# js43o/HifiDiff

Hardware: AMD Instinct MI355X
Metric: faces/sec (whole node), 16→128 1000-step reverse diffusion, batch 64 (higher is better)
Workload: dtype bf16

## Files before the change

hifidiff_amd/csrc/hd_xcd.hpp:

```cpp
#pragma once
#include <type_traits>
#ifndef HD_XCD_ROWS
#define HD_XCD_ROWS 0
#endif
#if HD_XCD_ROWS
#define HD_XCD_KERNEL xcd_rows_stage_kernel
#define HD_XCD_LAUNCH launch_xcd_rows_stage
#else
#define HD_XCD_KERNEL xcd_stage_kernel
#define HD_XCD_LAUNCH launch_xcd_stage
#endif

#include "hd_gemm.hpp"
#include "hd_stage_api.hpp"

#ifndef HD_XS_W0
#define HD_XS_W0 0
#endif
#ifndef HD_XS_READY
#define HD_XS_READY 1
#endif
#ifndef HD_XS_PUBFIRST
#define HD_XS_PUBFIRST 1
#endif
#ifndef HD_XS_WNT
#define HD_XS_WNT 0
#endif

#pragma clang fp contract(off)

namespace hd {

template <int C_, int HW_>
struct XcdCfg {
    static constexpr int C = C_, HW = HW_;
    static constexpr int R = XS_FACES * HW;
    static constexpr int NT = C / 32;
    static constexpr int RSPLIT = XS_GROUP_WG / NT;
    static constexpr int RCU = R / RSPLIT;
    static constexpr int WMW = RCU / 32;
    static constexpr int WK = 8 / WMW;
    static constexpr int CPW = C / 64 / WK;
    static constexpr int KS = C / 16;
    static constexpr int FCU = RCU / HW;
    static constexpr int S = (HW == 4) ? 2 : (HW == 16) ? 4 : (HW == 64) ? 8 : (HW == 256) ? 16 : 1;
    static constexpr int TPR = XS_THREADS / RCU;
    static constexpr int NIT = RCU * 32 / XS_THREADS;
    static constexpr int A_WAVE = 32 * LDS_ROW;
    static constexpr bool kStoresFirst = C_ >= 1024;
    static_assert(RSPLIT * NT == XS_GROUP_WG && WMW * WK == 8 && CPW == 2 && S * S == HW, "geometry");
    static_assert(RCU / S * 32 == XS_THREADS, "one (channel, image row) item per thread in the depthwise epilogue");
    static_assert(TPR * 4 >= NT, "partials per thread");
};

template <int C, int HW, int GBF = 1>
struct XLds {
    typedef XcdCfg<C, HW> K;
    char stage[K::WK * K::RCU * 32 * 2 * 4];
    float xt[K::RCU * 32], yt[K::RCU * 32];
    unsigned short gt[K::RCU * 32];
    float rs[(K::RCU / K::S) * 32];
    float pl[XS_FACES * 32];
    float2 stats[K::RCU];
    float gb[GBF * 2 * C];
    float dwc[22 * 32];
    XBlockW blk[XS_MAXBLK];
    unsigned base, local, abort, pad_;
};

typedef __attribute__((address_space(1))) unsigned xs_gu32;
typedef unsigned xs_u32x4 __attribute__((ext_vector_type(4)));
typedef unsigned xs_u32x2 __attribute__((ext_vector_type(2)));

__device__ __forceinline__ unsigned xs_xcc_id() {
    unsigned v;
    asm volatile("s_getreg_b32 %0, hwreg(HW_REG_XCC_ID)" : "=s"(v));
    return v & 0xfu;
}
__device__ __forceinline__ uint4 xs_ldg_u4(const uint4* p) {
#if HD_XS_WNT
    const xs_u32x4 v = __builtin_nontemporal_load(reinterpret_cast<__attribute__((address_space(1))) const xs_u32x4*>((unsigned long long)p));
#else
    const xs_u32x4 v = *reinterpret_cast<__attribute__((address_space(1))) const xs_u32x4*>((unsigned long long)p);
#endif
    return make_uint4(v.x, v.y, v.z, v.w);
}
__device__ __forceinline__ float xs_ldg_f(const float* p) { return *reinterpret_cast<__attribute__((address_space(1))) const float*>((unsigned long long)p); }
__device__ __forceinline__ float4 xs_ldg_f4(const float* p) {
    typedef float f4v __attribute__((ext_vector_type(4)));
    const f4v v = *reinterpret_cast<__attribute__((address_space(1))) const f4v*>((unsigned long long)p);
    return make_float4(v.x, v.y, v.z, v.w);
}
__device__ __forceinline__ void xs_ready(float& x) {
#if HD_XS_READY
    asm volatile("" : "+v"(x));
#endif
}
__device__ __forceinline__ void xs_lds_barrier() { asm volatile("s_waitcnt lgkmcnt(0)\n\ts_barrier" ::: "memory"); }

#ifdef HD_STAMPS
#define HD_XSTAMP(i) do { if (p.stamps && tid == 0) p.stamps[((size_t)ph * 256 + blockIdx.x) * 8 + (i)] = __builtin_amdgcn_s_memrealtime(); } while (0)
#else
#define HD_XSTAMP(i) do { } while (0)
#endif

template <int C, int HW>
__global__ __launch_bounds__(XS_THREADS) void HD_XCD_KERNEL(const XStageP p) {
    typedef XcdCfg<C, HW> K;
    __shared__ __attribute__((aligned(16))) XLds<C, HW, HD_XCD_ROWS ? XcdCfg<C, HW>::FCU : 1> L;
    const int tid = threadIdx.x, lane = tid & 63, wave = __builtin_amdgcn_readfirstlane(tid >> 6);
    const int group = blockIdx.x & 7, rank = blockIdx.x >> 3;
    const int face_g0 = group * XS_FACES;
    if (face_g0 >= p.B) return;
    const int ct = rank % K::NT, rsp = rank / K::NT;
    const int M = p.B * HW;
    const int row0 = face_g0 * HW + rsp * K::RCU;
    const int face0 = row0 / HW;
    const int wm = wave / K::WK, wk = wave - wm * K::WK;
    const int c0 = wk * K::CPW;
    const int kq = lane & 7;
    const int col = ct * 32 + (tid & 31);

    {
        const unsigned* src = reinterpret_cast<const unsigned*>(p.blocks);
        unsigned* dst = reinterpret_cast<unsigned*>(L.blk);
        for (int i = tid; i < p.nblocks * (int)(sizeof(XBlockW) / 4); i += XS_THREADS) dst[i] = src[i];
        if (tid == 0) L.abort = __hip_atomic_load((xs_gu32*)p.abort_dev, __ATOMIC_RELAXED, __HIP_MEMORY_SCOPE_AGENT);
    }
    xs_lds_barrier();

#ifdef HD_STAMPS
    const size_t act_bytes = p.dbg_no_a ? 0 : (size_t)M * C * 2;
#else
    const size_t act_bytes = (size_t)M * C * 2;
#endif
    const __amdgpu_buffer_rsrc_t rs_Xb = __builtin_amdgcn_make_buffer_rsrc(p.Xb, 0, (int)act_bytes, 0x00020000);
    const __amdgpu_buffer_rsrc_t rs_Yb = __builtin_amdgcn_make_buffer_rsrc(p.Yb, 0, (int)act_bytes, 0x00020000);
    const __amdgpu_buffer_rsrc_t rs_G = __builtin_amdgcn_make_buffer_rsrc(p.G, 0, (int)act_bytes, 0x00020000);
    const __amdgpu_buffer_rsrc_t rs_P16 = __builtin_amdgcn_make_buffer_rsrc(p.pooled16, 0, p.B * C * 2, 0x00020000);
    const __amdgpu_buffer_rsrc_t rs_sx = __builtin_amdgcn_make_buffer_rsrc(p.sx, 0, M * K::NT * 8, 0x00020000);
    const __amdgpu_buffer_rsrc_t rs_sy = __builtin_amdgcn_make_buffer_rsrc(p.sy, 0, M * K::NT * 8, 0x00020000);

    uint4 bq[K::CPW][4][2];
    xs_u32x4 aq[K::CPW][4];
    f32x16_t acc[2];

    auto load_w_chunk = [&](const uint4* W, auto pair_c, auto d_c) __attribute__((always_inline)) {
        constexpr bool PAIR = decltype(pair_c)::value;
        constexpr int d = decltype(d_c)::value;
#ifdef HD_STAMPS
        if (p.dbg_no_w) return;
#endif
        const uint4* Wl = W + lane;
#pragma unroll
        for (int ss = 0; ss < 4; ++ss) {
            bq[d][ss][0] = xs_ldg_u4(Wl + ((size_t)ct * K::KS + (c0 + d) * 4 + ss) * 64);
            if (PAIR) bq[d][ss][1] = xs_ldg_u4(Wl + ((size_t)(ct + K::NT) * K::KS + (c0 + d) * 4 + ss) * 64);
        }
    };
    auto load_w = [&](const uint4* W, auto pair_c) __attribute__((always_inline)) {
        load_w_chunk(W, pair_c, std::integral_constant<int, 0>());
        load_w_chunk(W, pair_c, std::integral_constant<int, 1>());
    };
    auto load_a = [&](const __amdgpu_buffer_rsrc_t& rs) __attribute__((always_inline)) {
#pragma unroll
        for (int d = 0; d < K::CPW; ++d)
#pragma unroll
            for (int u = 0; u < 4; ++u) {
                const int gr = row0 + wm * 32 + (lane >> 3) + 8 * u;
                const int r = gr < M ? gr : 0;
                aq[d][u] = __builtin_amdgcn_raw_buffer_load_b128(rs, (r * C + (c0 + d) * 64 + 8 * kq) * 2, 0, 16);
            }
    };
    char* sA = L.stage + wave * K::A_WAVE;
    const int a_lane_off = (lane & 31) * LDS_ROW + (lane >> 5) * 16;
    auto zero_acc = [&]() __attribute__((always_inline)) {
#pragma unroll
        for (int tn = 0; tn < 2; ++tn)
#pragma unroll
            for (int i = 0; i < 16; ++i) acc[tn][i] = 0.f;
    };
    auto chunk_mma = [&](int d, auto pair_c) __attribute__((always_inline)) {
        constexpr bool PAIR = decltype(pair_c)::value;
        __builtin_amdgcn_wave_barrier();
#pragma unroll
        for (int ss = 0; ss < 4; ++ss) {
            const bf16x8_t a = *reinterpret_cast<const bf16x8_t*>(sA + a_lane_off + ss * 32);
            acc[0] = __builtin_amdgcn_mfma_f32_32x32x16_bf16(a, __builtin_bit_cast(bf16x8_t, bq[d][ss][0]), acc[0], 0, 0, 0);
            if (PAIR) acc[1] = __builtin_amdgcn_mfma_f32_32x32x16_bf16(a, __builtin_bit_cast(bf16x8_t, bq[d][ss][1]), acc[1], 0, 0, 0);
        }
        __builtin_amdgcn_wave_barrier();
    };
    auto gemm_plain = [&](auto pair_c) __attribute__((always_inline)) {
        zero_acc();
#pragma unroll
        for (int d = 0; d < K::CPW; ++d) {
#pragma unroll
            for (int u = 0; u < 4; ++u) {
                const int gr = row0 + wm * 32 + (lane >> 3) + 8 * u;
                const xs_u32x4 v = gr < M ? aq[d][u] : (xs_u32x4){0u, 0u, 0u, 0u};
                *reinterpret_cast<xs_u32x4*>(sA + ((lane >> 3) + 8 * u) * LDS_ROW + 16 * kq) = v;
            }
            chunk_mma(d, pair_c);
        }
    };
    auto gemm_ln = [&]() __attribute__((always_inline)) {
        zero_acc();
        f32x2_t rsv[4], muv[4];
#pragma unroll
        for (int u = 0; u < 4; ++u) {
            float2 s = L.stats[wm * 32 + (lane >> 3) + 8 * u];
            asm volatile("s_waitcnt lgkmcnt(0)\n\ts_nop 3" : "+v"(s.x), "+v"(s.y));
            const float mu = -s.x * s.y;
            rsv[u] = (f32x2_t){s.y, s.y}; muv[u] = (f32x2_t){mu, mu};
        }
#pragma unroll
        for (int d = 0; d < K::CPW; ++d) {
            const int k = (c0 + d) * 64 + 8 * kq;
            f32x2_t g[4], b[4];
#if !HD_XCD_ROWS
#pragma unroll
            for (int i = 0; i < 4; ++i) {
                g[i] = *reinterpret_cast<const f32x2_t*>(&L.gb[k + 2 * i]);
                b[i] = *reinterpret_cast<const f32x2_t*>(&L.gb[C + k + 2 * i]);
            }
#endif
#pragma unroll
            for (int u = 0; u < 4; ++u) {
#if HD_XCD_ROWS
                {
                    const float* gbf = &L.gb[((wm * 32 + (lane >> 3) + 8 * u) / HW) * 2 * C];
#pragma unroll
                    for (int i = 0; i < 4; ++i) {
                        g[i] = *reinterpret_cast<const f32x2_t*>(&gbf[k + 2 * i]);
                        b[i] = *reinterpret_cast<const f32x2_t*>(&gbf[C + k + 2 * i]);
                    }
                }
#endif
                const unsigned w[4] = {aq[d][u].x, aq[d][u].y, aq[d][u].z, aq[d][u].w};
                unsigned o[4];
#pragma unroll
                for (int i = 0; i < 4; ++i) {
                    const f32x2_t x = {__uint_as_float(w[i] << 16), __uint_as_float(w[i] & 0xffff0000u)};
                    o[i] = pack2(__builtin_elementwise_fma(__builtin_elementwise_fma(x, rsv[u], muv[u]), g[i], b[i]));
                }
                *reinterpret_cast<xs_u32x4*>(sA + ((lane >> 3) + 8 * u) * LDS_ROW + 16 * kq) = (xs_u32x4){o[0], o[1], o[2], o[3]};
            }
            chunk_mma(d, std::true_type());
        }
    };
    float* red = reinterpret_cast<float*>(L.stage);
    auto to_red = [&](auto pair_c) __attribute__((always_inline)) {
        constexpr int TNT = decltype(pair_c)::value ? 2 : 1;
        constexpr int TILE_F = K::RCU * 32 * TNT;
        xs_lds_barrier();
#pragma unroll
        for (int tn = 0; tn < TNT; ++tn)
#pragma unroll
            for (int i = 0; i < 16; ++i) {
                const int r = wm * 32 + (i & 3) + 8 * (i >> 2) + 4 * (lane >> 5);
                red[wk * TILE_F + (tn * K::RCU + r) * 32 + (lane & 31)] = acc[tn][i];
            }
        xs_lds_barrier();
    };
    float2 ln_ps[4];
    float4 ln_g = make_float4(0.f, 0.f, 0.f, 0.f), ln_b = ln_g;
#if HD_XCD_ROWS
    int ln_film_off = 0;
#endif
    auto ln_issue = [&](const __amdgpu_buffer_rsrc_t& rs, int film_bias_off) __attribute__((always_inline)) {
        constexpr int TPR = K::TPR;
        const int rl = tid / TPR, part = tid % TPR, row = row0 + rl;
        const bool rv = row < M;
#pragma unroll
        for (int i = 0; i < 4; ++i) {
            const int j = part + i * TPR;
            ln_ps[i] = make_float2(0.f, -1.f);
            if (rv && j < K::NT) {
                const xs_u32x2 raw = __builtin_amdgcn_raw_buffer_load_b64(rs, (row * K::NT + j) * 8, 0, 16);
                ln_ps[i] = make_float2(__uint_as_float(raw.x), __uint_as_float(raw.y));
            }
        }
        static_assert(C <= XS_THREADS * 4, "one float4 of gain and bias per thread");
        const int k = tid * 4;
#if HD_XCD_ROWS
        ln_film_off = film_bias_off;
        (void)k;
#else
        if (k < C) {
            ln_b = *reinterpret_cast<const float4*>(p.film + film_bias_off + k);
            ln_g = *reinterpret_cast<const float4*>(p.film + film_bias_off + C + k);
        }
#endif
    };
    auto ln_finish = [&]() __attribute__((always_inline)) {
        constexpr int TPR = K::TPR;
        const int rl = tid / TPR, part = tid % TPR;
        const bool rv = row0 + rl < M;
        const int k = tid * 4;
#if HD_XCD_ROWS
        (void)ln_g; (void)ln_b; (void)k;
        for (int q = tid; q < K::FCU * (C / 4); q += XS_THREADS) {
            const int f = q / (C / 4), kk = (q - f * (C / 4)) * 4;
            const int face = (face0 + f) < p.B ? face0 + f : 0;
            const float* src = p.film + (size_t)face * p.film_face_stride + ln_film_off;
            *reinterpret_cast<float4*>(&L.gb[f * 2 * C + kk]) = *reinterpret_cast<const float4*>(src + C + kk);
            *reinterpret_cast<float4*>(&L.gb[f * 2 * C + C + kk]) = *reinterpret_cast<const float4*>(src + kk);
        }
#else
        if (k < C) {
            *reinterpret_cast<float4*>(&L.gb[k]) = ln_g;
            *reinterpret_cast<float4*>(&L.gb[C + k]) = ln_b;
        }
#endif
        auto row_sum = [](float v) __attribute__((always_inline)) {
            if (TPR > 1) v += dpp_mov<0xB1>(v);
            if (TPR > 2) v += dpp_mov<0x4E>(v);
            if (TPR > 4) v += dpp_mov<0x141>(v);
            if (TPR > 8) v += dpp_mov<0x140>(v);
            return v;
        };
        float sm = 0.f;
#pragma unroll
        for (int i = 0; i < 4; ++i) sm += ln_ps[i].y >= 0.f ? ln_ps[i].x : 0.f;
        const float inv_np = 1.0f / (float)K::NT;
        const float mean = row_sum(sm) * inv_np;
        const float cnt = 32.f;
        float q = 0.f;
#pragma unroll
        for (int i = 0; i < 4; ++i) {
            const float d = ln_ps[i].x - mean;
            q += ln_ps[i].y >= 0.f ? fmaf(cnt * d, d, ln_ps[i].y) : 0.f;
        }
        const float var = row_sum(q) * (inv_np / cnt);
        if (part == 0) L.stats[rl] = make_float2(mean, rv ? __frsqrt_rn(var + p.ln_eps) : 0.f);
        xs_lds_barrier();
    };
    bool local = false;
    auto st128 = [&](const __amdgpu_buffer_rsrc_t& rs, int off, uint4 v) __attribute__((always_inline)) {
        const xs_u32x4 x = {v.x, v.y, v.z, v.w};
        if (local) __builtin_amdgcn_raw_buffer_store_b128(x, rs, off, 0, 0);
        else __builtin_amdgcn_raw_buffer_store_b128(x, rs, off, 0, 16);
    };
    auto st64 = [&](const __amdgpu_buffer_rsrc_t& rs, int off, float2 v) __attribute__((always_inline)) {
        const xs_u32x2 x = {__float_as_uint(v.x), __float_as_uint(v.y)};
        if (local) __builtin_amdgcn_raw_buffer_store_b64(x, rs, off, 0, 0);
        else __builtin_amdgcn_raw_buffer_store_b64(x, rs, off, 0, 16);
    };
    xs_gu32* flags = (xs_gu32*)(p.flags + group * 32);
    unsigned base = 0;
    bool dead = false;
    auto publish = [&](int ph) __attribute__((always_inline)) {
        asm volatile("s_waitcnt vmcnt(0)" ::: "memory");
        if (lane == 0) {
            if (local) __hip_atomic_store(flags + rank, base + (unsigned)ph + 1u, __ATOMIC_RELAXED, __HIP_MEMORY_SCOPE_WORKGROUP);
            else __hip_atomic_store(flags + rank, base + (unsigned)ph + 1u, __ATOMIC_RELAXED, __HIP_MEMORY_SCOPE_AGENT);
        }
    };
    auto wait_phase = [&](int ph) __attribute__((always_inline)) {
        if (wave == 0) {
            const unsigned want = base + (unsigned)ph + 1u;
            for (unsigned spins = 0;; ++spins) {
                const unsigned v = lane < XS_GROUP_WG ? __hip_atomic_load(flags + lane, __ATOMIC_RELAXED, __HIP_MEMORY_SCOPE_AGENT) : want;
                const bool inject = p.test_abort > 0 && ph + 1 == p.test_abort && group == 0;
                if (!inject && __all((int)(v - want) >= 0)) break;
                if (spins > XS_SPINS || inject) {
                    if (lane == 0) {
                        L.abort = 1u;
                        __hip_atomic_store((xs_gu32*)p.abort_dev, 0x100u + (unsigned)ph, __ATOMIC_RELAXED, __HIP_MEMORY_SCOPE_AGENT);
                        __hip_atomic_store((xs_gu32*)p.tmo, 0x100u + (unsigned)ph, __ATOMIC_RELAXED, __HIP_MEMORY_SCOPE_SYSTEM);
                    }
                    break;
                }
                __builtin_amdgcn_s_sleep(1);
            }
        }
        xs_lds_barrier();
        dead = L.abort != 0u;
    };
    float2* st_out = L.stats;

    load_w(L.blk[0].w1, std::true_type());
    if (wave == 0) {
        xs_gu32* gs = (xs_gu32*)(p.gstate + group * 32);
        xs_gu32* hello = (xs_gu32*)(p.hello + group * 32);
        const unsigned n = __hip_atomic_load(gs, __ATOMIC_RELAXED, __HIP_MEMORY_SCOPE_AGENT);
        const unsigned xcc = xs_xcc_id();
        const unsigned mine = ((n + 1u) << 4) | xcc;
        if (lane == 0) __hip_atomic_store(hello + rank, mine, __ATOMIC_RELAXED, __HIP_MEMORY_SCOPE_AGENT);
        bool same = false;
        for (unsigned spins = 0;; ++spins) {
            const unsigned v = lane < XS_GROUP_WG ? __hip_atomic_load(hello + lane, __ATOMIC_RELAXED, __HIP_MEMORY_SCOPE_AGENT) : mine;
            if (__all((v >> 4) == (n + 1u))) { same = __all((v & 15u) == xcc); break; }
            if (spins > XS_SPINS) {
                if (lane == 0) {
                    L.abort = 1u;
                    __hip_atomic_store((xs_gu32*)p.abort_dev, 0x80u, __ATOMIC_RELAXED, __HIP_MEMORY_SCOPE_AGENT);
                    __hip_atomic_store((xs_gu32*)p.tmo, 0x80u, __ATOMIC_RELAXED, __HIP_MEMORY_SCOPE_SYSTEM);
                }
                break;
            }
            __builtin_amdgcn_s_sleep(1);
        }
        if (lane == 0) { L.base = n * 64u; L.local = (same && !p.force_global) ? 1u : 0u; }
    }
    for (int u = tid; u < K::RCU * 8; u += XS_THREADS) {
        const int r = u >> 3, q4 = u & 7;
        float4 v = make_float4(0.f, 0.f, 0.f, 0.f);
        if (row0 + r < M) v = *reinterpret_cast<const float4*>(p.X + (size_t)(row0 + r) * C + ct * 32 + q4 * 4);
        *reinterpret_cast<float4*>(&L.xt[r * 32 + q4 * 4]) = v;
    }
    xs_lds_barrier();
    if (L.abort) return;
    base = L.base; local = L.local != 0u;

    const int P = 5 * p.nblocks;
    const int P_run = (p.phase_limit > 0 && p.phase_limit < P) ? p.phase_limit : P;

    for (int blk = 0; blk < p.nblocks; ++blk) {
        const XBlockW& B = L.blk[blk];
        {
            const int ph = 5 * blk;
            if (ph >= P_run) break;
            HD_XSTAMP(0);
            if (ph > 0) { wait_phase(ph - 1); if (dead) return; }
            HD_XSTAMP(1);
            ln_issue(rs_sx, B.film_off);
            if (HD_XS_W0 == 0 && ph > 0 && wave == 0) load_w(B.w1, std::true_type());
            load_a(rs_Xb);
            float dwc[2];
#pragma unroll
            for (int i = 0; i < 2; ++i) {
                const int e = tid + i * XS_THREADS, k = e >> 5, cc = ct * 32 + (e & 31);
                dwc[i] = 0.f;
                if (k < 18) dwc[i] = xs_ldg_f(B.dw_w + (size_t)(k % 9) * 2 * C + cc + (k >= 9 ? C : 0));
                else if (k < 20) dwc[i] = xs_ldg_f(B.dw_b + cc + (k == 19 ? C : 0));
                else if (k < 22) dwc[i] = xs_ldg_f(B.b1 + cc + (k == 21 ? C : 0));
            }
            ln_finish();
            gemm_ln();
            if ((wave != 0 || HD_XS_W0 >= 2) && ph + 1 < P_run) load_w_chunk(B.wsca, std::false_type(), std::integral_constant<int, 0>());
            if (HD_XS_W0 == 2 && wave == 0 && ph + 1 < P_run) load_w_chunk(B.wsca, std::false_type(), std::integral_constant<int, 1>());
            HD_XSTAMP(2);
#pragma unroll
            for (int i = 0; i < 2; ++i) { const int e = tid + i * XS_THREADS; if (e < 22 * 32) L.dwc[e] = dwc[i]; }
            to_red(std::true_type());
            HD_XSTAMP(6);
            constexpr int TILE_F = K::RCU * 32 * 2;
            float dw_wa[9], dw_wb[9];
            const int jc = tid & 31;
#pragma unroll
            for (int t = 0; t < 9; ++t) { dw_wa[t] = L.dwc[t * 32 + jc]; dw_wb[t] = L.dwc[(9 + t) * 32 + jc]; }
            const float dw_ba = L.dwc[18 * 32 + jc], dw_bb = L.dwc[19 * 32 + jc], b1a = L.dwc[20 * 32 + jc], b1b = L.dwc[21 * 32 + jc];
            for (int e = tid; e < K::RCU * 32; e += XS_THREADS) {
                float va = b1a, vb = b1b;
#pragma unroll
                for (int w = 0; w < K::WK; ++w) { va += red[w * TILE_F + e]; vb += red[w * TILE_F + K::RCU * 32 + e]; }
                red[e] = va; red[K::RCU * 32 + e] = vb;
            }
            xs_lds_barrier();
            {
                const int j = tid & 31, rr = tid >> 5;
                constexpr int ls = (K::S == 2) ? 1 : (K::S == 4) ? 2 : (K::S == 8) ? 3 : (K::S == 16) ? 4 : 0;
                const int p0 = rr << ls;
                const int y = (p0 & (HW - 1)) >> ls;
                const float rsum = dw_gate_row<K::S>(red + j, red + K::RCU * 32 + j, p0, y > 0, y < K::S - 1, dw_wa, dw_wb, dw_ba, dw_bb,
                                                     L.gt + p0 * 32 + j, 32, true, K::S);
                L.rs[rr * 32 + j] = rsum;
            }
            xs_lds_barrier();
            if (tid < K::FCU * 32) {
                const int f = tid >> 5, j = tid & 31;
                float sacc = 0.f;
#pragma unroll
                for (int r = 0; r < K::S; ++r) sacc += L.rs[(f * K::S + r) * 32 + j];
                L.pl[f * 32 + j] = sacc / (float)HW;
            }
            xs_lds_barrier();
            if constexpr (!K::kStoresFirst) { if (wave != 0 && ph + 1 < P_run) load_w_chunk(B.wsca, std::false_type(), std::integral_constant<int, 1>()); }
            HD_XSTAMP(3);
            if (wave == 0) {
                if (lane < K::FCU * 4) {
                    const int f = lane >> 2, q4 = lane & 3;
                    if (face0 + f < p.B) {
                        st128(rs_P16, ((face0 + f) * C + ct * 32 + q4 * 8) * 2, pack8(&L.pl[f * 32 + q4 * 8]));
                        if (p.pooled) {
                            *reinterpret_cast<float4*>(p.pooled + (size_t)(face0 + f) * C + ct * 32 + q4 * 8) = *reinterpret_cast<const float4*>(&L.pl[f * 32 + q4 * 8]);
                            *reinterpret_cast<float4*>(p.pooled + (size_t)(face0 + f) * C + ct * 32 + q4 * 8 + 4) = *reinterpret_cast<const float4*>(&L.pl[f * 32 + q4 * 8 + 4]);
                        }
                    }
                }
                HD_XSTAMP(4);
            }
#if HD_XS_PUBFIRST
            if (wave == 0) publish(ph);
#endif
            if constexpr (K::kStoresFirst) xs_lds_barrier();
            if constexpr (K::kStoresFirst) { if (wave != 0 && ph + 1 < P_run) load_w_chunk(B.wsca, std::false_type(), std::integral_constant<int, 1>()); }
#if !HD_XS_PUBFIRST
            if (wave == 0) publish(ph);
#endif
            if (HD_XS_W0 == 1 && wave == 0 && ph + 1 < P_run) load_w(B.wsca, std::false_type());
            if (HD_XS_W0 == 3 && wave == 0 && ph + 1 < P_run) load_w_chunk(B.wsca, std::false_type(), std::integral_constant<int, 1>());
            HD_XSTAMP(5);
        }
        {
            const int ph = 5 * blk + 1;
            if (ph >= P_run) break;
            HD_XSTAMP(0);
            wait_phase(ph - 1); if (dead) return;
            if (HD_XS_W0 == 0 && wave == 0) load_w(B.wsca, std::false_type());
            HD_XSTAMP(1);
            float bsca = xs_ldg_f(B.bsca + col);
            zero_acc();
            if (wm == 0) {
                xs_u32x4 pa[K::CPW];
                const int f = lane >> 3;
                const bool fv = f < K::FCU && face0 + f < p.B;
#pragma unroll
                for (int d = 0; d < K::CPW; ++d)
                    pa[d] = __builtin_amdgcn_raw_buffer_load_b128(rs_P16, ((fv ? face0 + f : 0) * C + (c0 + d) * 64 + 8 * kq) * 2, 0, 16);
                for (int i = lane; i < 24 * LDS_ROW / 16; i += 64) reinterpret_cast<uint4*>(sA + 8 * LDS_ROW)[i] = make_uint4(0, 0, 0, 0);
#pragma unroll
                for (int d = 0; d < K::CPW; ++d) {
                    *reinterpret_cast<xs_u32x4*>(sA + f * LDS_ROW + 16 * kq) = fv ? pa[d] : (xs_u32x4){0u, 0u, 0u, 0u};
                    chunk_mma(d, std::false_type());
                }
            }
            xs_ready(bsca);
            if ((wave != 0 || HD_XS_W0 >= 2) && ph + 1 < P_run) load_w_chunk(B.w3, std::false_type(), std::integral_constant<int, 0>());
            if (HD_XS_W0 == 2 && wave == 0 && ph + 1 < P_run) load_w_chunk(B.w3, std::false_type(), std::integral_constant<int, 1>());
            HD_XSTAMP(2);
            xs_lds_barrier();
            if (wm == 0) {
#pragma unroll
                for (int i = 0; i < 16; ++i) {
                    const int r = (i & 3) + 8 * (i >> 2) + 4 * (lane >> 5);
                    if (r < XS_FACES) red[wk * (XS_FACES * 32) + r * 32 + (lane & 31)] = acc[0][i];
                }
            }
            xs_lds_barrier();
            HD_XSTAMP(6);
            if (tid < K::FCU * 32) {
                float v = bsca;
#pragma unroll
                for (int w = 0; w < K::WK; ++w) v += red[w * (XS_FACES * 32) + tid];
                L.pl[tid] = v;
            }
            xs_lds_barrier();
            if constexpr (!K::kStoresFirst) { if (wave != 0 && ph + 1 < P_run) load_w_chunk(B.w3, std::false_type(), std::integral_constant<int, 1>()); }
            HD_XSTAMP(3);
            if (wave == 0) {
                for (int u = lane; u < K::RCU * 4; u += 64) {
                    const int r = u >> 2, q4 = u & 3;
                    if (row0 + r < M) {
                        const uint4 g = *reinterpret_cast<const uint4*>(&L.gt[r * 32 + q4 * 8]);
                        float v[8];
                        unpack8(g, v);
                        const float* sp = &L.pl[(r / HW) * 32 + q4 * 8];
#pragma unroll
                        for (int i = 0; i < 8; ++i) v[i] *= sp[i];
                        st128(rs_G, ((row0 + r) * C + ct * 32 + q4 * 8) * 2, pack8(v));
                    }
                }
                if (p.S) for (int e = lane; e < K::FCU * 32; e += 64) if (face0 + (e >> 5) < p.B) p.S[(size_t)(face0 + (e >> 5)) * C + ct * 32 + (e & 31)] = L.pl[e];
                HD_XSTAMP(4);
            }
#if HD_XS_PUBFIRST
            if (wave == 0) publish(ph);
#endif
            if constexpr (K::kStoresFirst) xs_lds_barrier();
            if constexpr (K::kStoresFirst) { if (wave != 0 && ph + 1 < P_run) load_w_chunk(B.w3, std::false_type(), std::integral_constant<int, 1>()); }
#if !HD_XS_PUBFIRST
            if (wave == 0) publish(ph);
#endif
            if (HD_XS_W0 == 1 && wave == 0 && ph + 1 < P_run) load_w(B.w3, std::false_type());
            if (HD_XS_W0 == 3 && wave == 0 && ph + 1 < P_run) load_w_chunk(B.w3, std::false_type(), std::integral_constant<int, 1>());
            HD_XSTAMP(5);
        }
        {
            const int ph = 5 * blk + 2;
            if (ph >= P_run) break;
            HD_XSTAMP(0);
            wait_phase(ph - 1); if (dead) return;
            if (HD_XS_W0 == 0 && wave == 0) load_w(B.w3, std::false_type());
            HD_XSTAMP(1);
            load_a(rs_G);
            float b3 = xs_ldg_f(B.b3 + col), beta = xs_ldg_f(B.beta + col);
            gemm_plain(std::false_type());
            xs_ready(b3); xs_ready(beta);
            if ((wave != 0 || HD_XS_W0 >= 2) && ph + 1 < P_run) load_w_chunk(B.w4, std::true_type(), std::integral_constant<int, 0>());
            if (HD_XS_W0 == 2 && wave == 0 && ph + 1 < P_run) load_w_chunk(B.w4, std::true_type(), std::integral_constant<int, 1>());
            HD_XSTAMP(2);
            to_red(std::false_type());
            HD_XSTAMP(6);
            constexpr int TILE_F = K::RCU * 32;
            float v[K::NIT];
#pragma unroll
            for (int it = 0; it < K::NIT; ++it) {
                const int e = it * XS_THREADS + tid;
                float s = 0.f;
#pragma unroll
                for (int w = 0; w < K::WK; ++w) s += red[w * TILE_F + e];
                v[it] = fmaf(s + b3, beta, L.xt[e]);
                if (row0 + (e >> 5) >= M) v[it] = 0.f;
                L.yt[e] = v[it];
            }
            {
                float2 ms[K::NIT];
#pragma unroll
                for (int it = 0; it < K::NIT; ++it) ms[it] = halfwave_mean_m2(v[it]);
                if ((tid & 31) == kStatLane) {
#pragma unroll
                    for (int it = 0; it < K::NIT; ++it) st_out[(it * XS_THREADS + tid) >> 5] = ms[it];
                }
            }
            xs_lds_barrier();
            if constexpr (!K::kStoresFirst) { if (wave != 0 && ph + 1 < P_run) load_w_chunk(B.w4, std::true_type(), std::integral_constant<int, 1>()); }
            HD_XSTAMP(3);
            if (wave == 0) {
                for (int u = lane; u < K::RCU * 4; u += 64) {
                    const int r = u >> 2, q4 = u & 3;
                    if (row0 + r < M) st128(rs_Yb, ((row0 + r) * C + ct * 32 + q4 * 8) * 2, pack8(&L.yt[r * 32 + q4 * 8]));
                }
                for (int r = lane; r < K::RCU; r += 64) if (row0 + r < M) st64(rs_sy, ((row0 + r) * K::NT + ct) * 8, st_out[r]);
                HD_XSTAMP(4);
            }
#if HD_XS_PUBFIRST
            if (wave == 0) publish(ph);
#endif
            if constexpr (K::kStoresFirst) xs_lds_barrier();
            if constexpr (K::kStoresFirst) { if (wave != 0 && ph + 1 < P_run) load_w_chunk(B.w4, std::true_type(), std::integral_constant<int, 1>()); }
#if !HD_XS_PUBFIRST
            if (wave == 0) publish(ph);
#endif
            if (HD_XS_W0 == 1 && wave == 0 && ph + 1 < P_run) load_w(B.w4, std::true_type());
            if (HD_XS_W0 == 3 && wave == 0 && ph + 1 < P_run) load_w_chunk(B.w4, std::true_type(), std::integral_constant<int, 1>());
            HD_XSTAMP(5);
        }
        {
            const int ph = 5 * blk + 3;
            if (ph >= P_run) break;
            HD_XSTAMP(0);
            wait_phase(ph - 1); if (dead) return;
            HD_XSTAMP(1);
            ln_issue(rs_sy, B.film_off + 2 * C);
            if (HD_XS_W0 == 0 && wave == 0) load_w(B.w4, std::true_type());
            load_a(rs_Yb);
            float b4a = xs_ldg_f(B.b4 + col), b4b = xs_ldg_f(B.b4 + col + C);
            ln_finish();
            gemm_ln();
            xs_ready(b4a); xs_ready(b4b);
            if ((wave != 0 || HD_XS_W0 >= 2) && ph + 1 < P_run) load_w_chunk(B.w5, std::false_type(), std::integral_constant<int, 0>());
            if (HD_XS_W0 == 2 && wave == 0 && ph + 1 < P_run) load_w_chunk(B.w5, std::false_type(), std::integral_constant<int, 1>());
            HD_XSTAMP(2);
            to_red(std::true_type());
            HD_XSTAMP(6);
            constexpr int TILE_F = K::RCU * 32 * 2;
#pragma unroll
            for (int it = 0; it < K::NIT; ++it) {
                const int e = it * XS_THREADS + tid;
                float v1 = 0.f, v2 = 0.f;
#pragma unroll
                for (int w = 0; w < K::WK; ++w) { v1 += red[w * TILE_F + e]; v2 += red[w * TILE_F + K::RCU * 32 + e]; }
                L.gt[e] = f32_to_bf16_bits((v1 + b4a) * (v2 + b4b));
            }
            xs_lds_barrier();
            if constexpr (!K::kStoresFirst) { if (wave != 0 && ph + 1 < P_run) load_w_chunk(B.w5, std::false_type(), std::integral_constant<int, 1>()); }
            HD_XSTAMP(3);
            if (wave == 0) {
                for (int u = lane; u < K::RCU * 4; u += 64) {
                    const int r = u >> 2, q4 = u & 3;
                    if (row0 + r < M) st128(rs_G, ((row0 + r) * C + ct * 32 + q4 * 8) * 2, *reinterpret_cast<const uint4*>(&L.gt[r * 32 + q4 * 8]));
                }
                HD_XSTAMP(4);
            }
#if HD_XS_PUBFIRST
            if (wave == 0) publish(ph);
#endif
            if constexpr (K::kStoresFirst) xs_lds_barrier();
            if constexpr (K::kStoresFirst) { if (wave != 0 && ph + 1 < P_run) load_w_chunk(B.w5, std::false_type(), std::integral_constant<int, 1>()); }
#if !HD_XS_PUBFIRST
            if (wave == 0) publish(ph);
#endif
            if (HD_XS_W0 == 1 && wave == 0 && ph + 1 < P_run) load_w(B.w5, std::false_type());
            if (HD_XS_W0 == 3 && wave == 0 && ph + 1 < P_run) load_w_chunk(B.w5, std::false_type(), std::integral_constant<int, 1>());
            HD_XSTAMP(5);
        }
        {
            const int ph = 5 * blk + 4;
            if (ph >= P_run) break;
            HD_XSTAMP(0);
            wait_phase(ph - 1); if (dead) return;
            if (HD_XS_W0 == 0 && wave == 0) load_w(B.w5, std::false_type());
            HD_XSTAMP(1);
            load_a(rs_G);
            float b5 = xs_ldg_f(B.b5 + col), gamma = xs_ldg_f(B.gamma + col);
            const bool last = (ph == P_run - 1);
            const bool gated = last && ph == P - 1 && p.outg16 != nullptr;
            gemm_plain(std::false_type());
            xs_ready(b5); xs_ready(gamma);
            if ((wave != 0 || HD_XS_W0 >= 2) && !last) load_w_chunk(L.blk[blk + 1].w1, std::true_type(), std::integral_constant<int, 0>());
            if (HD_XS_W0 == 2 && wave == 0 && !last) load_w_chunk(L.blk[blk + 1].w1, std::true_type(), std::integral_constant<int, 1>());
            HD_XSTAMP(2);
            to_red(std::false_type());
            HD_XSTAMP(6);
            constexpr int TILE_F = K::RCU * 32;
            float v[K::NIT];
#pragma unroll
            for (int it = 0; it < K::NIT; ++it) {
                const int e = it * XS_THREADS + tid;
                float s = 0.f;
#pragma unroll
                for (int w = 0; w < K::WK; ++w) s += red[w * TILE_F + e];
                v[it] = fmaf(s + b5, gamma, L.yt[e]);
                if (row0 + (e >> 5) >= M) v[it] = 0.f;
                L.xt[e] = v[it];
            }
            if (!gated) {
                float2 ms[K::NIT];
#pragma unroll
                for (int it = 0; it < K::NIT; ++it) ms[it] = halfwave_mean_m2(v[it]);
                if ((tid & 31) == kStatLane) {
#pragma unroll
                    for (int it = 0; it < K::NIT; ++it) st_out[(it * XS_THREADS + tid) >> 5] = ms[it];
                }
            }
            xs_lds_barrier();
            if constexpr (!K::kStoresFirst) { if (wave != 0 && !last) load_w_chunk(L.blk[blk + 1].w1, std::true_type(), std::integral_constant<int, 1>()); }
            HD_XSTAMP(3);
            if (wave == 0 && !gated) {
                for (int u = lane; u < K::RCU * 4; u += 64) {
                    const int r = u >> 2, q4 = u & 3;
                    if (row0 + r < M) st128(rs_Xb, ((row0 + r) * C + ct * 32 + q4 * 8) * 2, pack8(&L.xt[r * 32 + q4 * 8]));
                }
                for (int r = lane; r < K::RCU; r += 64) if (row0 + r < M) st64(rs_sx, ((row0 + r) * K::NT + ct) * 8, st_out[r]);
            }
            if (last) {
                int row0e = row0;
                int tide = tid;
                asm volatile("" : "+s"(row0e), "+v"(tide));
                if (tide < K::RCU * 4) {
                    const int r = tide >> 2, q4 = tide & 3;
                    const int row = row0e + r;
                    if (row < M) {
                        const float* xv = &L.xt[r * 32 + q4 * 8];
                        float* xo = p.X + (size_t)row * C + ct * 32 + q4 * 8;
                        *reinterpret_cast<float4*>(xo) = *reinterpret_cast<const float4*>(xv);
                        *reinterpret_cast<float4*>(xo + 4) = *reinterpret_cast<const float4*>(xv + 4);
                        if (gated) {
                            float gv[8];
                            const float gsr = p.gate_s[row];
                            const size_t o = (size_t)row * C + ct * 32 + q4 * 8;
                            const float* gc = p.gate_c + (size_t)(row / HW) * C + ct * 32 + q4 * 8;
#pragma unroll
                            for (int i = 0; i < 8; ++i) {
                                const float a = p.add_src ? p.add_src[o + i] : 0.f;
                                const float g = 1.0f + gc[i] + gsr;
                                gv[i] = (xv[i] + a) * g;
                            }
                            *reinterpret_cast<uint4*>(p.outg16 + o) = pack8(gv);
                        }
                    }
                }
            } else if (wave == 0) {
                HD_XSTAMP(4);
            }
#if HD_XS_PUBFIRST
            if (wave == 0 && !last) publish(ph);
#endif
            if constexpr (K::kStoresFirst) xs_lds_barrier();
            if constexpr (K::kStoresFirst) { if (wave != 0 && !last) load_w_chunk(L.blk[blk + 1].w1, std::true_type(), std::integral_constant<int, 1>()); }
#if !HD_XS_PUBFIRST
            if (wave == 0 && !last) publish(ph);
#endif
            if (HD_XS_W0 == 1 && wave == 0 && !last) load_w(L.blk[blk + 1].w1, std::true_type());
            if (HD_XS_W0 == 3 && wave == 0 && !last) load_w_chunk(L.blk[blk + 1].w1, std::true_type(), std::integral_constant<int, 1>());
            HD_XSTAMP(5);
        }
    }
    if (rank == 0 && tid == 0) {
        xs_gu32* gs = (xs_gu32*)(p.gstate + group * 32);
        __hip_atomic_store(gs, base / 64u + 1u, __ATOMIC_RELAXED, __HIP_MEMORY_SCOPE_AGENT);
    }
}

template <int C, int HW>
inline hipError_t HD_XCD_LAUNCH(const XStageP& p, hipStream_t s) {
    if (p.B < 1 || p.B > XS_GROUPS * XS_FACES || p.nblocks < 1 || p.nblocks > XS_MAXBLK) return hipErrorInvalidValue;
    hipLaunchKernelGGL((HD_XCD_KERNEL<C, HW>), dim3(XS_GROUPS * XS_GROUP_WG), dim3(XS_THREADS), 0, s, p);
    return hipGetLastError();
}

}

#pragma clang fp contract(fast)
```

Before: 67.81.

## Prefetch wave-0 weight fragments into LDS via async global-to-LDS DMA

```diff
diff --git a/hifidiff_amd/csrc/hd_xcd.hpp b/hifidiff_amd/csrc/hd_xcd.hpp
--- a/hifidiff_amd/csrc/hd_xcd.hpp
+++ b/hifidiff_amd/csrc/hd_xcd.hpp
@@ -53,7 +53,7 @@
     static_assert(TPR * 4 >= NT, "partials per thread");
 };
 
-template <int C, int HW, int GBF = 1>
+template <int C, int HW, int GBF = 1, bool W0F = false>
 struct XLds {
     typedef XcdCfg<C, HW> K;
     char stage[K::WK * K::RCU * 32 * 2 * 4];
@@ -66,6 +66,7 @@
     float dwc[22 * 32];
     XBlockW blk[XS_MAXBLK];
     unsigned base, local, abort, pad_;
+    uint4 w0[W0F ? 2 * 16 * 64 : 1];
 };
 
 typedef __attribute__((address_space(1))) unsigned xs_gu32;
@@ -97,6 +98,12 @@
 #endif
 }
 __device__ __forceinline__ void xs_lds_barrier() { asm volatile("s_waitcnt lgkmcnt(0)\n\ts_barrier" ::: "memory"); }
+__device__ __forceinline__ unsigned xs_lds_addr(const void* p) { return (unsigned)(unsigned long long)(const __attribute__((address_space(3))) void*)p; }
+__device__ __forceinline__ void xs_dma16(const uint4* gsrc_lane, unsigned lds_dst) {
+    unsigned keep;
+    asm volatile("s_mov_b32 %0, m0\n\ts_mov_b32 m0, %2\n\ts_nop 0\n\tglobal_load_lds_dwordx4 %1, off\n\ts_mov_b32 m0, %0"
+                 : "=&s"(keep) : "v"(gsrc_lane), "s"(lds_dst) : "memory");
+}
 
 #ifdef HD_STAMPS
 #define HD_XSTAMP(i) do { if (p.stamps && tid == 0) p.stamps[((size_t)ph * 256 + blockIdx.x) * 8 + (i)] = __builtin_amdgcn_s_memrealtime(); } while (0)
@@ -107,7 +114,10 @@
 template <int C, int HW>
 __global__ __launch_bounds__(XS_THREADS) void HD_XCD_KERNEL(const XStageP p) {
     typedef XcdCfg<C, HW> K;
-    __shared__ __attribute__((aligned(16))) XLds<C, HW, HD_XCD_ROWS ? XcdCfg<C, HW>::FCU : 1> L;
+    constexpr bool kW0Lds = HD_XS_W0 == 4 && C >= 1024 && !HD_XCD_ROWS;
+    constexpr int W0 = HD_XS_W0 == 4 ? (kW0Lds ? 4 : 0) : HD_XS_W0;
+    constexpr bool kW0Early = W0 == 2 || W0 == 3;
+    __shared__ __attribute__((aligned(16))) XLds<C, HW, HD_XCD_ROWS ? XcdCfg<C, HW>::FCU : 1, kW0Lds> L;
     const int tid = threadIdx.x, lane = tid & 63, wave = __builtin_amdgcn_readfirstlane(tid >> 6);
     const int group = blockIdx.x & 7, rank = blockIdx.x >> 3;
     const int face_g0 = group * XS_FACES;
@@ -162,6 +172,35 @@
         load_w_chunk(W, pair_c, std::integral_constant<int, 0>());
         load_w_chunk(W, pair_c, std::integral_constant<int, 1>());
     };
+    const unsigned w0_lds = xs_lds_addr(L.w0);
+    auto w0_request = [&](const uint4* W, auto pair_c, int par) __attribute__((always_inline)) {
+        constexpr bool PAIR = decltype(pair_c)::value;
+        constexpr int NF = PAIR ? 16 : 8;
+#ifdef HD_STAMPS
+        if (p.dbg_no_w) return;
+#endif
+        const uint4* Wl = W + lane;
+#pragma unroll
+        for (int j = 0; j < (NF + 6) / 7; ++j) {
+            const int f = wave - 1 + 7 * j;
+            if (f < NF) {
+                const int ks = PAIR ? (f >> 1) : f, h = PAIR ? (f & 1) : 0;
+                xs_dma16(Wl + ((size_t)(ct + h * K::NT) * K::KS + ks) * 64, w0_lds + (unsigned)((par * 16 + f) * 1024));
+            }
+        }
+    };
+    auto w0_fill = [&](auto pair_c, int par) __attribute__((always_inline)) {
+        constexpr bool PAIR = decltype(pair_c)::value;
+        const uint4* src = L.w0 + par * 16 * 64 + lane;
+#pragma unroll
+        for (int d = 0; d < 2; ++d)
+#pragma unroll
+            for (int ss = 0; ss < 4; ++ss) {
+                bq[d][ss][0] = src[(PAIR ? 2 * (d * 4 + ss) : d * 4 + ss) * 64];
+                if (PAIR) bq[d][ss][1] = src[(2 * (d * 4 + ss) + 1) * 64];
+            }
+    };
+    auto xs_drain = [&]() __attribute__((always_inline)) { if constexpr (kW0Lds) asm volatile("s_waitcnt vmcnt(0)" ::: "memory"); };
     auto load_a = [&](const __amdgpu_buffer_rsrc_t& rs) __attribute__((always_inline)) {
 #pragma unroll
         for (int d = 0; d < K::CPW; ++d)
@@ -357,7 +396,8 @@
             else __hip_atomic_store(flags + rank, base + (unsigned)ph + 1u, __ATOMIC_RELAXED, __HIP_MEMORY_SCOPE_AGENT);
         }
     };
-    auto wait_phase = [&](int ph) __attribute__((always_inline)) {
+    auto wait_phase = [&](int ph, auto nw_c) __attribute__((always_inline)) {
+        if constexpr (kW0Lds) { if (wave != 0) asm volatile("s_waitcnt vmcnt(%0)" :: "n"(decltype(nw_c)::value) : "memory"); }
         if (wave == 0) {
             const unsigned want = base + (unsigned)ph + 1u;
             for (unsigned spins = 0;; ++spins) {
@@ -423,10 +463,11 @@
             const int ph = 5 * blk;
             if (ph >= P_run) break;
             HD_XSTAMP(0);
-            if (ph > 0) { wait_phase(ph - 1); if (dead) return; }
+            if (ph > 0) { wait_phase(ph - 1, std::integral_constant<int, 16>()); if (dead) { xs_drain(); return; } }
             HD_XSTAMP(1);
             ln_issue(rs_sx, B.film_off);
-            if (HD_XS_W0 == 0 && ph > 0 && wave == 0) load_w(B.w1, std::true_type());
+            if (W0 == 0 && ph > 0 && wave == 0) load_w(B.w1, std::true_type());
+            if constexpr (kW0Lds) { if (ph > 0 && wave == 0) w0_fill(std::true_type(), ph & 1); }
             load_a(rs_Xb);
             float dwc[2];
 #pragma unroll
@@ -439,8 +480,9 @@
             }
             ln_finish();
             gemm_ln();
-            if ((wave != 0 || HD_XS_W0 >= 2) && ph + 1 < P_run) load_w_chunk(B.wsca, std::false_type(), std::integral_constant<int, 0>());
-            if (HD_XS_W0 == 2 && wave == 0 && ph + 1 < P_run) load_w_chunk(B.wsca, std::false_type(), std::integral_constant<int, 1>());
+            if constexpr (kW0Lds) { if (wave != 0 && ph + 1 < P_run) w0_request(B.wsca, std::false_type(), (ph + 1) & 1); }
+            if ((wave != 0 || kW0Early) && ph + 1 < P_run) load_w_chunk(B.wsca, std::false_type(), std::integral_constant<int, 0>());
+            if (W0 == 2 && wave == 0 && ph + 1 < P_run) load_w_chunk(B.wsca, std::false_type(), std::integral_constant<int, 1>());
             HD_XSTAMP(2);
 #pragma unroll
             for (int i = 0; i < 2; ++i) { const int e = tid + i * XS_THREADS; if (e < 22 * 32) L.dwc[e] = dwc[i]; }
@@ -500,16 +542,17 @@
 #if !HD_XS_PUBFIRST
             if (wave == 0) publish(ph);
 #endif
-            if (HD_XS_W0 == 1 && wave == 0 && ph + 1 < P_run) load_w(B.wsca, std::false_type());
-            if (HD_XS_W0 == 3 && wave == 0 && ph + 1 < P_run) load_w_chunk(B.wsca, std::false_type(), std::integral_constant<int, 1>());
+            if (W0 == 1 && wave == 0 && ph + 1 < P_run) load_w(B.wsca, std::false_type());
+            if (W0 == 3 && wave == 0 && ph + 1 < P_run) load_w_chunk(B.wsca, std::false_type(), std::integral_constant<int, 1>());
             HD_XSTAMP(5);
         }
         {
             const int ph = 5 * blk + 1;
             if (ph >= P_run) break;
             HD_XSTAMP(0);
-            wait_phase(ph - 1); if (dead) return;
-            if (HD_XS_W0 == 0 && wave == 0) load_w(B.wsca, std::false_type());
+            wait_phase(ph - 1, std::integral_constant<int, 8>()); if (dead) { xs_drain(); return; }
+            if (W0 == 0 && wave == 0) load_w(B.wsca, std::false_type());
+            if constexpr (kW0Lds) { if (wave == 0) w0_fill(std::false_type(), ph & 1); }
             HD_XSTAMP(1);
             float bsca = xs_ldg_f(B.bsca + col);
             zero_acc();
@@ -528,8 +571,9 @@
                 }
             }
             xs_ready(bsca);
-            if ((wave != 0 || HD_XS_W0 >= 2) && ph + 1 < P_run) load_w_chunk(B.w3, std::false_type(), std::integral_constant<int, 0>());
-            if (HD_XS_W0 == 2 && wave == 0 && ph + 1 < P_run) load_w_chunk(B.w3, std::false_type(), std::integral_constant<int, 1>());
+            if constexpr (kW0Lds) { if (wave != 0 && ph + 1 < P_run) w0_request(B.w3, std::false_type(), (ph + 1) & 1); }
+            if ((wave != 0 || kW0Early) && ph + 1 < P_run) load_w_chunk(B.w3, std::false_type(), std::integral_constant<int, 0>());
+            if (W0 == 2 && wave == 0 && ph + 1 < P_run) load_w_chunk(B.w3, std::false_type(), std::integral_constant<int, 1>());
             HD_XSTAMP(2);
             xs_lds_barrier();
             if (wm == 0) {
@@ -574,23 +618,25 @@
 #if !HD_XS_PUBFIRST
             if (wave == 0) publish(ph);
 #endif
-            if (HD_XS_W0 == 1 && wave == 0 && ph + 1 < P_run) load_w(B.w3, std::false_type());
-            if (HD_XS_W0 == 3 && wave == 0 && ph + 1 < P_run) load_w_chunk(B.w3, std::false_type(), std::integral_constant<int, 1>());
+            if (W0 == 1 && wave == 0 && ph + 1 < P_run) load_w(B.w3, std::false_type());
+            if (W0 == 3 && wave == 0 && ph + 1 < P_run) load_w_chunk(B.w3, std::false_type(), std::integral_constant<int, 1>());
             HD_XSTAMP(5);
         }
         {
             const int ph = 5 * blk + 2;
             if (ph >= P_run) break;
             HD_XSTAMP(0);
-            wait_phase(ph - 1); if (dead) return;
-            if (HD_XS_W0 == 0 && wave == 0) load_w(B.w3, std::false_type());
+            wait_phase(ph - 1, std::integral_constant<int, 8>()); if (dead) { xs_drain(); return; }
+            if (W0 == 0 && wave == 0) load_w(B.w3, std::false_type());
+            if constexpr (kW0Lds) { if (wave == 0) w0_fill(std::false_type(), ph & 1); }
             HD_XSTAMP(1);
             load_a(rs_G);
             float b3 = xs_ldg_f(B.b3 + col), beta = xs_ldg_f(B.beta + col);
             gemm_plain(std::false_type());
             xs_ready(b3); xs_ready(beta);
-            if ((wave != 0 || HD_XS_W0 >= 2) && ph + 1 < P_run) load_w_chunk(B.w4, std::true_type(), std::integral_constant<int, 0>());
-            if (HD_XS_W0 == 2 && wave == 0 && ph + 1 < P_run) load_w_chunk(B.w4, std::true_type(), std::integral_constant<int, 1>());
+            if constexpr (kW0Lds) { if (wave != 0 && ph + 1 < P_run) w0_request(B.w4, std::true_type(), (ph + 1) & 1); }
+            if ((wave != 0 || kW0Early) && ph + 1 < P_run) load_w_chunk(B.w4, std::true_type(), std::integral_constant<int, 0>());
+            if (W0 == 2 && wave == 0 && ph + 1 < P_run) load_w_chunk(B.w4, std::true_type(), std::integral_constant<int, 1>());
             HD_XSTAMP(2);
             to_red(std::false_type());
             HD_XSTAMP(6);
@@ -634,25 +680,27 @@
 #if !HD_XS_PUBFIRST
             if (wave == 0) publish(ph);
 #endif
-            if (HD_XS_W0 == 1 && wave == 0 && ph + 1 < P_run) load_w(B.w4, std::true_type());
-            if (HD_XS_W0 == 3 && wave == 0 && ph + 1 < P_run) load_w_chunk(B.w4, std::true_type(), std::integral_constant<int, 1>());
+            if (W0 == 1 && wave == 0 && ph + 1 < P_run) load_w(B.w4, std::true_type());
+            if (W0 == 3 && wave == 0 && ph + 1 < P_run) load_w_chunk(B.w4, std::true_type(), std::integral_constant<int, 1>());
             HD_XSTAMP(5);
         }
         {
             const int ph = 5 * blk + 3;
             if (ph >= P_run) break;
             HD_XSTAMP(0);
-            wait_phase(ph - 1); if (dead) return;
+            wait_phase(ph - 1, std::integral_constant<int, 16>()); if (dead) { xs_drain(); return; }
             HD_XSTAMP(1);
             ln_issue(rs_sy, B.film_off + 2 * C);
-            if (HD_XS_W0 == 0 && wave == 0) load_w(B.w4, std::true_type());
+            if (W0 == 0 && wave == 0) load_w(B.w4, std::true_type());
+            if constexpr (kW0Lds) { if (wave == 0) w0_fill(std::true_type(), ph & 1); }
             load_a(rs_Yb);
             float b4a = xs_ldg_f(B.b4 + col), b4b = xs_ldg_f(B.b4 + col + C);
             ln_finish();
             gemm_ln();
             xs_ready(b4a); xs_ready(b4b);
-            if ((wave != 0 || HD_XS_W0 >= 2) && ph + 1 < P_run) load_w_chunk(B.w5, std::false_type(), std::integral_constant<int, 0>());
-            if (HD_XS_W0 == 2 && wave == 0 && ph + 1 < P_run) load_w_chunk(B.w5, std::false_type(), std::integral_constant<int, 1>());
+            if constexpr (kW0Lds) { if (wave != 0 && ph + 1 < P_run) w0_request(B.w5, std::false_type(), (ph + 1) & 1); }
+            if ((wave != 0 || kW0Early) && ph + 1 < P_run) load_w_chunk(B.w5, std::false_type(), std::integral_constant<int, 0>());
+            if (W0 == 2 && wave == 0 && ph + 1 < P_run) load_w_chunk(B.w5, std::false_type(), std::integral_constant<int, 1>());
             HD_XSTAMP(2);
             to_red(std::true_type());
             HD_XSTAMP(6);
@@ -683,16 +731,17 @@
 #if !HD_XS_PUBFIRST
             if (wave == 0) publish(ph);
 #endif
-            if (HD_XS_W0 == 1 && wave == 0 && ph + 1 < P_run) load_w(B.w5, std::false_type());
-            if (HD_XS_W0 == 3 && wave == 0 && ph + 1 < P_run) load_w_chunk(B.w5, std::false_type(), std::integral_constant<int, 1>());
+            if (W0 == 1 && wave == 0 && ph + 1 < P_run) load_w(B.w5, std::false_type());
+            if (W0 == 3 && wave == 0 && ph + 1 < P_run) load_w_chunk(B.w5, std::false_type(), std::integral_constant<int, 1>());
             HD_XSTAMP(5);
         }
         {
             const int ph = 5 * blk + 4;
             if (ph >= P_run) break;
             HD_XSTAMP(0);
-            wait_phase(ph - 1); if (dead) return;
-            if (HD_XS_W0 == 0 && wave == 0) load_w(B.w5, std::false_type());
+            wait_phase(ph - 1, std::integral_constant<int, 8>()); if (dead) { xs_drain(); return; }
+            if (W0 == 0 && wave == 0) load_w(B.w5, std::false_type());
+            if constexpr (kW0Lds) { if (wave == 0) w0_fill(std::false_type(), ph & 1); }
             HD_XSTAMP(1);
             load_a(rs_G);
             float b5 = xs_ldg_f(B.b5 + col), gamma = xs_ldg_f(B.gamma + col);
@@ -700,8 +749,9 @@
             const bool gated = last && ph == P - 1 && p.outg16 != nullptr;
             gemm_plain(std::false_type());
             xs_ready(b5); xs_ready(gamma);
-            if ((wave != 0 || HD_XS_W0 >= 2) && !last) load_w_chunk(L.blk[blk + 1].w1, std::true_type(), std::integral_constant<int, 0>());
-            if (HD_XS_W0 == 2 && wave == 0 && !last) load_w_chunk(L.blk[blk + 1].w1, std::true_type(), std::integral_constant<int, 1>());
+            if constexpr (kW0Lds) { if (wave != 0 && !last) w0_request(L.blk[blk + 1].w1, std::true_type(), (ph + 1) & 1); }
+            if ((wave != 0 || kW0Early) && !last) load_w_chunk(L.blk[blk + 1].w1, std::true_type(), std::integral_constant<int, 0>());
+            if (W0 == 2 && wave == 0 && !last) load_w_chunk(L.blk[blk + 1].w1, std::true_type(), std::integral_constant<int, 1>());
             HD_XSTAMP(2);
             to_red(std::false_type());
             HD_XSTAMP(6);
@@ -774,11 +824,12 @@
 #if !HD_XS_PUBFIRST
             if (wave == 0 && !last) publish(ph);
 #endif
-            if (HD_XS_W0 == 1 && wave == 0 && !last) load_w(L.blk[blk + 1].w1, std::true_type());
-            if (HD_XS_W0 == 3 && wave == 0 && !last) load_w_chunk(L.blk[blk + 1].w1, std::true_type(), std::integral_constant<int, 1>());
+            if (W0 == 1 && wave == 0 && !last) load_w(L.blk[blk + 1].w1, std::true_type());
+            if (W0 == 3 && wave == 0 && !last) load_w_chunk(L.blk[blk + 1].w1, std::true_type(), std::integral_constant<int, 1>());
             HD_XSTAMP(5);
         }
     }
+    xs_drain();
     if (rank == 0 && tid == 0) {
         xs_gu32* gs = (xs_gu32*)(p.gstate + group * 32);
         __hip_atomic_store(gs, base / 64u + 1u, __ATOMIC_RELAXED, __HIP_MEMORY_SCOPE_AGENT);
```

New measurement: 67.13. 0.99x the previous value.
